# Gorilla-Lab-SCUT/DCL-Net

Hardware: AMD Instinct MI355X
Metric: frames/sec DCL_Net.forward @ YCB-V bs32 (higher is better)
Workload: dtype f32 (exact 3xbf16-split products on the bf16 MFMA, f32 accumulate)

## Files before the change

dcl-net_amd/csrc/linear_split.hip:

```cpp
#include <hip/hip_runtime.h>
#include "common.h"

namespace {

typedef float sp_f32x16 __attribute__((ext_vector_type(16)));
typedef float sp_f32x2 __attribute__((ext_vector_type(2)));
typedef __bf16 sp_bf16x2 __attribute__((ext_vector_type(2)));
typedef __bf16 sp_bf16x8 __attribute__((ext_vector_type(8)));
typedef unsigned sp_u32x4 __attribute__((ext_vector_type(4)));
typedef __attribute__((address_space(3))) void sp_lds_void_t;

constexpr int kSpKC = 16;
constexpr int kSpBM = 256, kSpBN = 128;
constexpr int kSpA = kSpBM * kSpKC * 4;
constexpr int kSpP = kSpBN * kSpKC * 2;
constexpr int kSpB = 3 * kSpP;
constexpr int kSpST = kSpA + kSpB;

__device__ __forceinline__ unsigned sp_lds_addr(const void *p) {
  return __builtin_amdgcn_readfirstlane((unsigned)(size_t)(sp_lds_void_t *)p);
}
__device__ __forceinline__ void sp_glds16(unsigned voff, const void *sbase, unsigned lds_byte_addr) {
  unsigned keep;
  asm volatile("s_mov_b32 %0, m0\n\ts_mov_b32 m0, %3\n\ts_nop 0\n\tglobal_load_lds_dwordx4 %1, %2\n\ts_mov_b32 m0, %0"
               : "=&s"(keep) : "v"(voff), "s"(sbase), "s"(lds_byte_addr) : "memory");
}
__device__ __forceinline__ unsigned sp_cvt2(float a, float b) {
  const sp_f32x2 v = {a, b};
  return __builtin_bit_cast(unsigned, __builtin_convertvector(v, sp_bf16x2));
}
__device__ __forceinline__ void sp_split2(float x0, float x1, unsigned &h, unsigned &m, unsigned &l) {
  h = sp_cvt2(x0, x1);
  float r0 = x0 - __uint_as_float(h << 16);
  asm volatile("" : "+v"(r0));
  float r1 = x1 - __uint_as_float(h & 0xffff0000u);
  asm volatile("" : "+v"(r1));
  m = sp_cvt2(r0, r1);
  float s0 = r0 - __uint_as_float(m << 16);
  asm volatile("" : "+v"(s0));
  float s1 = r1 - __uint_as_float(m & 0xffff0000u);
  asm volatile("" : "+v"(s1));
  l = sp_cvt2(s0, s1);
}
__device__ __forceinline__ sp_bf16x8 sp_bf(sp_u32x4 v) { return __builtin_bit_cast(sp_bf16x8, v); }

struct LinSplitArgs {
  const float *x;
  const unsigned char *planes;
  const float *bias;
  float *y;
  long long ldx, ldy;
  int M, N, K, relu;
  const float *roww;
  int rows_per_crop;
  long long w_stride;
  float *part;
  const float *b3;
  long long ldp;
  int xcd_remap;
};

__device__ __forceinline__ int sp_rowmap(int e, int h) { return (e & 3) + 8 * (e >> 2) + 4 * h; }

__global__ __launch_bounds__(256) void k_split_weight(const float *__restrict__ Wt, long long ldw, int K, int N, unsigned *__restrict__ planes) {
  const int ntn = (N + kSpBN - 1) / kSpBN;
  const long long pieces = (long long)(K / kSpKC) * ntn * kSpBN * 2;
  for (long long i = blockIdx.x * 256ll + threadIdx.x; i < pieces; i += (long long)gridDim.x * 256) {
    const int hs = (int)(i & 1), c = (int)((i >> 1) & (kSpBN - 1));
    const long long ct = i >> 8;
    const int kc = (int)(ct / ntn), tn = (int)(ct - (long long)kc * ntn);
    const int hh = hs ^ ((c >> 3) & 1), col = tn * kSpBN + c, k0 = kc * kSpKC + 8 * hh;
    unsigned h[4], m[4], l[4];
#pragma unroll
    for (int e = 0; e < 4; ++e) {
      const float w0 = col < N ? Wt[(size_t)(k0 + 2 * e) * ldw + col] : 0.0f, w1 = col < N ? Wt[(size_t)(k0 + 2 * e + 1) * ldw + col] : 0.0f;
      sp_split2(w0, w1, h[e], m[e], l[e]);
    }
    unsigned *dst = planes + (size_t)ct * (kSpB / 4) + (size_t)(c * 2 + hs) * 4;
#pragma unroll
    for (int e = 0; e < 4; ++e) { dst[e] = h[e]; dst[kSpP / 4 + e] = m[e]; dst[2 * (kSpP / 4) + e] = l[e]; }
  }
}

template <int EPI>
__global__ __launch_bounds__(256, 2) void k_linear_split(const LinSplitArgs a) {
  extern __shared__ __attribute__((aligned(16))) unsigned char sp_lds[];
  const int ntn = (a.N + kSpBN - 1) / kSpBN, ntm = (a.M + kSpBM - 1) / kSpBM, tiles = ntm * ntn;
  int t_lo, t_hi, t_stride;
  {
    const int id = blockIdx.x, nwg = gridDim.x;
    if ((a.xcd_remap & 1) && (nwg & 7) == 0) {
      const int xq = tiles >> 3, xr = tiles & 7, xcd = id & 7;
      const int x_lo = xcd < xr ? xcd * (xq + 1) : xr * (xq + 1) + (xcd - xr) * xq;
      t_lo = x_lo + (id >> 3);
      t_hi = x_lo + xq + (xcd < xr ? 1 : 0);
      t_stride = nwg >> 3;
    } else {
      t_lo = id; t_hi = tiles; t_stride = nwg;
    }
  }
  const int tid = threadIdx.x, lane = tid & 63, wave = __builtin_amdgcn_readfirstlane(tid >> 6);
  const int r = lane & 31, h = lane >> 5;
  const int nchunks = a.K / kSpKC;
  const int whatif = a.xcd_remap >> 1;
  const unsigned lds0 = sp_lds_addr(sp_lds);
  const size_t bstep = (size_t)ntn * kSpB;

  const int asw = (r >> 2) & 3;
  const unsigned char *afrag = sp_lds + (wave * 64 + r) * 64;
  const unsigned char *bfrag = sp_lds + kSpA + r * 32 + ((h ^ ((r >> 3) & 1)) << 4);

  for (int tile = t_lo; tile < t_hi; tile += t_stride) {
    const int tm = tile / ntn, tn = tile - tm * ntn;
    const int row0 = tm * kSpBM, col0 = tn * kSpBN;
    unsigned aoff[4];
#pragma unroll
    for (int i = 0; i < 4; ++i) {
      const int row = wave * 64 + i * 16 + (lane >> 2);
      const int p = (lane & 3) ^ ((row >> 2) & 3);
      const int srow = min(row0 + row, a.M - 1) - row0;
      aoff[i] = (unsigned)(((long long)srow * a.ldx + 4 * p) * 4);
    }
    const unsigned boff = (unsigned)tid * 16u;
    const float *abase = a.x + (size_t)row0 * a.ldx;
    const unsigned char *bbase = a.planes + (size_t)tn * kSpB;
    auto issue_piece = [&](int k, int stage) {
      const unsigned s0 = lds0 + (unsigned)(stage * kSpST);
      if (k < 3) sp_glds16(boff + (unsigned)(k * 4096), bbase, s0 + (unsigned)(kSpA + k * 4096 + wave * 1024));
      else sp_glds16(aoff[k - 3], abase, s0 + (unsigned)((wave * 64 + (k - 3) * 16) * 64));
      if (k == 6) { abase += kSpKC; bbase += bstep; }
    };
    auto issue = [&](int stage) {
#pragma unroll
      for (int k = 0; k < 7; ++k) issue_piece(k, stage);
    };
    sp_f32x16 acc[2][4];
#pragma unroll
    for (int i = 0; i < 2; ++i)
#pragma unroll
      for (int j = 0; j < 4; ++j)
#pragma unroll
        for (int e = 0; e < 16; ++e) acc[i][j][e] = 0.0f;

    dcl_lds_barrier();
    if constexpr (EPI == 1) {
      float *wl = reinterpret_cast<float *>(sp_lds + 2 * kSpST);
      const int row = row0 + tid, crop = row / a.rows_per_crop;
      wl[tid] = row < a.M ? a.roww[(size_t)crop * a.w_stride + (row - crop * a.rows_per_crop)] : 0.0f;
    }
    issue(0);
    asm volatile("s_waitcnt vmcnt(0)" ::: "memory");
    for (int c = 0; c < nchunks; ++c) {
      const int st = c & 1;
      asm volatile("s_waitcnt lgkmcnt(0)" ::: "memory");
      __builtin_amdgcn_s_barrier();
      const bool more = c + 1 < nchunks;
      const unsigned char *sa = afrag + st * kSpST, *sb = bfrag + st * kSpST;
      float4 av[2][2];
      sp_u32x4 ap[2][3], bp[4][3];
      auto read_a = [&](int i) {
#pragma unroll
        for (int q = 0; q < 2; ++q) av[i][q] = *reinterpret_cast<const float4 *>(sa + i * 32 * 64 + (((2 * h + q) ^ asw) << 4));
      };
      auto read_b = [&](int j) {
#pragma unroll
        for (int p = 0; p < 3; ++p) bp[j][p] = *reinterpret_cast<const sp_u32x4 *>(sb + p * kSpP + j * 32 * 32);
      };
      auto split_a = [&](int i, int part) {
        unsigned ph, pm, pl;
        const float4 v = av[i][part >> 1];
        if (part & 1) sp_split2(v.z, v.w, ph, pm, pl); else sp_split2(v.x, v.y, ph, pm, pl);
        ap[i][0][part] = ph; ap[i][1][part] = pm; ap[i][2][part] = pl;
      };
      read_a(0);
      read_b(0);
      read_a(1);
      if (more && !(whatif & 1)) issue(st ^ 1);
      __builtin_amdgcn_sched_barrier(0);
      if (!(whatif & 2)) {
#pragma unroll
        for (int part = 0; part < 4; ++part) split_a(0, part);
      } else {
#pragma unroll
        for (int p = 0; p < 3; ++p) ap[0][p] = sp_u32x4{__float_as_uint(av[0][0].x), __float_as_uint(av[0][0].y), __float_as_uint(av[0][1].x), __float_as_uint(av[0][1].y)};
      }
      read_b(1);
      __builtin_amdgcn_sched_barrier(0);
#pragma unroll
      for (int blk = 0; blk < 8; ++blk) {
        const int i = blk >> 2, j = blk & 3;
        acc[i][j] = __builtin_amdgcn_mfma_f32_32x32x16_bf16(sp_bf(ap[i][2]), sp_bf(bp[j][0]), acc[i][j], 0, 0, 0);
        acc[i][j] = __builtin_amdgcn_mfma_f32_32x32x16_bf16(sp_bf(ap[i][0]), sp_bf(bp[j][2]), acc[i][j], 0, 0, 0);
        acc[i][j] = __builtin_amdgcn_mfma_f32_32x32x16_bf16(sp_bf(ap[i][1]), sp_bf(bp[j][1]), acc[i][j], 0, 0, 0);
        acc[i][j] = __builtin_amdgcn_mfma_f32_32x32x16_bf16(sp_bf(ap[i][1]), sp_bf(bp[j][0]), acc[i][j], 0, 0, 0);
        acc[i][j] = __builtin_amdgcn_mfma_f32_32x32x16_bf16(sp_bf(ap[i][0]), sp_bf(bp[j][1]), acc[i][j], 0, 0, 0);
        acc[i][j] = __builtin_amdgcn_mfma_f32_32x32x16_bf16(sp_bf(ap[i][0]), sp_bf(bp[j][0]), acc[i][j], 0, 0, 0);
        if (blk < 4) {
          if (!(whatif & 2)) split_a(1, blk);
          else { ap[1][0][blk] = __float_as_uint(av[1][blk >> 1].x); ap[1][1][blk] = __float_as_uint(av[1][blk >> 1].y); ap[1][2][blk] = __float_as_uint(av[1][blk >> 1].z); }
        }
        if (blk < 2) read_b(blk + 2);
        __builtin_amdgcn_sched_barrier(0);
      }
      asm volatile("s_waitcnt vmcnt(0)" ::: "memory");
    }
    asm volatile("s_nop 15\n\ts_nop 7" ::: "memory");

    if constexpr (EPI == 0) {
      if (whatif & 4) continue;
      float *__restrict__ y = a.y;
      const bool whole = row0 + kSpBM <= a.M && col0 + kSpBN <= a.N;
      float bias[4];
#pragma unroll
      for (int j = 0; j < 4; ++j) {
        const int co = col0 + j * 32 + r;
        bias[j] = (a.bias && co < a.N) ? a.bias[co] : 0.0f;
      }
      if (whole) {
#pragma unroll
        for (int i = 0; i < 2; ++i)
#pragma unroll
          for (int j = 0; j < 4; ++j) {
            float *yp = y + (size_t)(row0 + wave * 64 + i * 32 + 4 * h) * a.ldy + (col0 + j * 32 + r);
#pragma unroll
            for (int e = 0; e < 16; ++e) {
              float v = acc[i][j][e] + bias[j];
              if (a.relu) v = fmaxf(v, 0.0f);
              __builtin_nontemporal_store(v, yp + (size_t)((e & 3) + 8 * (e >> 2)) * a.ldy);
            }
          }
      } else {
#pragma unroll
        for (int i = 0; i < 2; ++i)
#pragma unroll
          for (int j = 0; j < 4; ++j) {
            const int co = col0 + j * 32 + r;
#pragma unroll
            for (int e = 0; e < 16; ++e) {
              const int orow = row0 + wave * 64 + i * 32 + sp_rowmap(e, h);
              float v = acc[i][j][e] + bias[j];
              if (a.relu) v = fmaxf(v, 0.0f);
              if (orow < a.M && co < a.N) y[(size_t)orow * a.ldy + co] = v;
            }
          }
      }
    } else if constexpr (EPI == 3) {
      unsigned char *vp = reinterpret_cast<unsigned char *>(a.part);
      const int crop = row0 / a.rows_per_crop, key0 = row0 - crop * a.rows_per_crop;
#pragma unroll
      for (int j = 0; j < 4; ++j) {
        const int c = col0 + j * 32 + r;
        const float bias = (a.bias && c < a.N) ? a.bias[c] : 0.0f;
        const int hs = h ^ ((c >> 3) & 1);
#pragma unroll
        for (int i = 0; i < 2; ++i)
#pragma unroll
          for (int hf = 0; hf < 2; ++hf) {
            const long long ht = (long long)crop * a.ldp + ((key0 + wave * 64 + i * 32) >> 4) + hf;
// ... 51 lines not shown
            const float wv[4] = {w4.x, w4.y, w4.z, w4.w};
#pragma unroll
            for (int q = 0; q < 4; ++q) {
              float v = acc[i][j][4 * g4 + q] + bias;
              if (a.relu) v = fmaxf(v, 0.0f);
              s = __fmaf_rn(v, wv[q], s);
            }
          }
        s += __shfl_xor(s, 32, 64);
        if (h == 0) red[wave * kSpBN + cl] = s;
      }
      dcl_lds_barrier();
      {
        const int pt = tid >> 7, cl = tid & 127;
        if (col0 + cl < a.N && row0 + pt * 128 < a.M)
          a.part[(size_t)(2 * tm + pt) * a.ldp + col0 + cl] = red[(2 * pt) * kSpBN + cl] + red[(2 * pt + 1) * kSpBN + cl];
      }
    }
  }
}

DCL_HOOK_INT(g_sp_xcd, 1);

template <int EPI>
int launch_linear_split(const LinSplitArgs &a, hipStream_t stream) {
  const long long tiles = (long long)((a.M + kSpBM - 1) / kSpBM) * ((a.N + kSpBN - 1) / kSpBN);
  if (tiles > 0x7fffffffll) {
    dcl_set_error("dcl_linear_split_fwd: too many tiles");
    return DCL_EINVAL;
  }
  constexpr size_t lds = (size_t)2 * kSpST + (EPI == 1 ? (kSpBM + 4 * kSpBN) * sizeof(float) : 0);
  static bool attr_set = false;
  if (!attr_set) {
    (void)hipFuncSetAttribute((const void *)k_linear_split<EPI>, hipFuncAttributeMaxDynamicSharedMemorySize, (int)lds);
    attr_set = true;
  }
  hipLaunchKernelGGL((k_linear_split<EPI>), dim3((unsigned)tiles), dim3(256), lds, stream, a);
  return 0;
}

bool lin_split_ok(const float *x, int64_t ldx, const void *planes, int K) {
  return K >= kSpKC && K % kSpKC == 0 && ldx % 4 == 0 && ((size_t)x & 15) == 0 && ((size_t)planes & 15) == 0;
}

}

#ifdef DCL_DIAG
DCL_API void dcl_debug_linear_split_xcd_remap(int on) { g_sp_xcd = ((int)g_sp_xcd & ~1) | (on & 1); }
DCL_API void dcl_debug_linear_split_whatif(int bits) { g_sp_xcd = ((int)g_sp_xcd & 1) | (bits << 1); }
#endif

DCL_API int64_t dcl_linear_split_weight_bytes(int K, int N) {
  if (K <= 0 || N <= 0 || K % kSpKC) return 0;
  return (int64_t)(K / kSpKC) * ((N + kSpBN - 1) / kSpBN) * kSpB;
}

DCL_API int dcl_linear_split_weight(const float *Wt, int64_t ldw, int K, int N, void *planes, dclStream_t stream) {
  DCL_CHECK_ARG(Wt && planes && K > 0 && N > 0 && K % kSpKC == 0 && ldw >= N && ((size_t)planes & 15) == 0);
  const long long pieces = (long long)(K / kSpKC) * ((N + kSpBN - 1) / kSpBN) * kSpBN * 2;
  const unsigned grid = (unsigned)((pieces + 255) / 256 > 4096 ? 4096 : (pieces + 255) / 256);
  hipLaunchKernelGGL(k_split_weight, dim3(grid), dim3(256), 0, (hipStream_t)stream, Wt, (long long)ldw, K, N, (unsigned *)planes);
  DCL_LAUNCH_CHECK();
  return 0;
}

DCL_API int dcl_linear_split_fwd(const float *x, int64_t ldx, const void *planes, const float *bias, float *y, int64_t ldy, int M, int N,
                                 int K, int relu, dclStream_t stream) {
  DCL_CHECK_ARG(M >= 0 && N > 0 && K > 0 && x && planes && y && ldx >= K && ldy >= N);
  DCL_CHECK_ARG(lin_split_ok(x, ldx, planes, K));
  if (M == 0) return 0;
  LinSplitArgs a{x, (const unsigned char *)planes, bias, y, ldx, ldy, M, N, K, relu, nullptr, 1, 0, nullptr, nullptr, 0, (int)g_sp_xcd};
  int rc = launch_linear_split<0>(a, (hipStream_t)stream);
  if (rc) return rc;
  DCL_LAUNCH_CHECK();
  return 0;
}

DCL_API int dcl_linear_split_pool_fwd(const float *x, int64_t ldx, const void *planes, const float *bias, const float *roww,
                                      int rows_per_crop, int64_t w_stride, float *part, int64_t ldp, int M, int N, int K, int relu,
                                      dclStream_t stream) {
  DCL_CHECK_ARG(M > 0 && N > 0 && K > 0 && x && planes && roww && part && ldx >= K && ldp >= N && rows_per_crop >= 1 && w_stride >= 0);
  DCL_CHECK_ARG(lin_split_ok(x, ldx, planes, K));
  LinSplitArgs a{x, (const unsigned char *)planes, bias, nullptr, ldx, 0, M, N, K, relu, roww, rows_per_crop, w_stride, part, nullptr, ldp,
                 (int)g_sp_xcd};
  int rc = launch_linear_split<1>(a, (hipStream_t)stream);
  if (rc) return rc;
  DCL_LAUNCH_CHECK();
  return 0;
}

DCL_API int dcl_linear_split_vpieces_fwd(const float *x, int64_t ldx, const void *planes, const float *bias, void *vplanes,
                                         int rows_per_crop, int M, int N, int K, int relu, dclStream_t stream) {
  DCL_CHECK_ARG(M > 0 && N > 0 && N <= 320 && N % 32 == 0 && K > 0 && x && planes && vplanes && ldx >= K && rows_per_crop > 0);
  DCL_CHECK_ARG(rows_per_crop % kSpBM == 0 && M % rows_per_crop == 0 && (((size_t)vplanes) & 15) == 0);
  DCL_CHECK_ARG(lin_split_ok(x, ldx, planes, K));
  LinSplitArgs a{x, (const unsigned char *)planes, bias, nullptr, ldx, 0, M, N, K, relu, nullptr, rows_per_crop, 0, (float *)vplanes, nullptr,
                 (long long)(rows_per_crop / 16), (int)g_sp_xcd};
  int rc = launch_linear_split<3>(a, (hipStream_t)stream);
  if (rc) return rc;
  DCL_LAUNCH_CHECK();
  return 0;
}

DCL_API int dcl_linear_split_rowdot_fwd(const float *x, int64_t ldx, const void *planes, const float *bias, const float *w3, int64_t ldw3,
                                        const float *b3, float *out, int M, int N, int K, dclStream_t stream) {
  DCL_CHECK_ARG(M >= 0 && N > 0 && N <= kSpBN && K > 0 && x && planes && w3 && b3 && out && ldx >= K && ldw3 >= 1);
  DCL_CHECK_ARG(lin_split_ok(x, ldx, planes, K));
  if (M == 0) return 0;
  LinSplitArgs a{x, (const unsigned char *)planes, bias, nullptr, ldx, 0, M, N, K, 1, w3, 1, ldw3, out, b3, 0, (int)g_sp_xcd};
  int rc = launch_linear_split<2>(a, (hipStream_t)stream);
  if (rc) return rc;
  DCL_LAUNCH_CHECK();
  return 0;
}
```

dcl-net_amd/models/DCL_Net.py:

```python
from functools import partial

import numpy as np
import torch
import torch.nn as nn

from .. import ops
from .. import spconv
from ..libs.pointgroup_ops.functions import pointgroup_ops
from .losses import losses
from .Modules import (Aligner, Backbone_SPCONV, BasicBlock_3DCONV, Head_MultiLayerPerceptron,
                      Ops_GetPointFeat_spconv)

HOST_TIMES = None
_QUEUE_SHIMS = []
SIDE_STREAM_PRIORITY = -1
_SIDE_STREAMS = {}
SCALE_LISTS = [2, 4, 6, 8]
VOXEL_NUM_LIMIT = [64, 64, 64]


def normalize_vector(v):
    return v / (torch.sqrt(v.pow(2).sum(1, keepdim=True)) + 1e-8)


def ortho9d2matrix(x_raw, y_raw, z_raw):
    if not (torch.is_grad_enabled() and (x_raw.requires_grad or y_raw.requires_grad or z_raw.requires_grad)):
        return ops.ortho9d_to_matrix(torch.cat([x_raw, y_raw, z_raw], dim=1))
    dev = x_raw.device
    m = torch.stack([normalize_vector(x_raw), normalize_vector(y_raw), normalize_vector(z_raw)], dim=2).cpu()
    U, _, Vh = torch.linalg.svd(m)
    ones = torch.ones(m.shape[0], dtype=m.dtype)
    sigma = torch.diag_embed(torch.stack([ones, ones, torch.det(U @ Vh)], dim=1))
    return (U @ sigma @ Vh).to(dev)


def _mlp3(dims):
    return Head_MultiLayerPerceptron(dims, ["relu", "relu", "none"], [False] * 3, [0.0] * 3)


def _fuser():
    return Head_MultiLayerPerceptron([512, 512, 512, 1024], ["relu"] * 3, [True] * 3, [0.0] * 3)


class Network(nn.Module):
    def __init__(self, cfg, mode="train", fused=True, graph_max_batch=8, async_inputs=False, graph_max_points=98304,
                 single_stream=False, pipeline_chunks=1, capture_graph=True, pair_features=None):
        super().__init__()
        self.single_stream = bool(single_stream)
        self._pair_features = pair_features
        self.pipeline_chunks = int(pipeline_chunks)
        self.capture_graph = bool(capture_graph)
        self.graph_max_batch = int(graph_max_batch)
        self.graph_max_points = int(graph_max_points)
        self.async_inputs = bool(async_inputs)
        self.voxelization_mode = cfg.voxelization_mode
        self.unit_voxel_extent = np.array(cfg.unit_voxel_extent)
        self.mode = mode
        self.fused = fused
        self.n_inp = cfg.n_inp
        self.n_tmp = cfg.n_tmp
        self.backbone_dims = [7, 16, 32, 32, 64, 64, 128, 128, 256]
        self.backbone_stride_layers = [1, 3, 5]
        self.backbone_inp = Backbone_SPCONV(self.backbone_dims, self.backbone_stride_layers, cfg.backbone)
        self.backbone_tmp = Backbone_SPCONV(self.backbone_dims, self.backbone_stride_layers, cfg.backbone)
        self.stage1_get_point_feats = Ops_GetPointFeat_spconv(SCALE_LISTS, self.unit_voxel_extent, VOXEL_NUM_LIMIT)
        block = partial(BasicBlock_3DCONV, size=1, bias=False, stride=1, padding=0, norm=True, act="relu", drop=0.0)
        for grp in ("1", "2"):
            for side in ("Xc", "Yo"):
                for kind, d_out in (("p", 256), ("m", 64)):
                    setattr(self, "disengage_%s_%s%s" % (side, kind, grp),
# ... 303 lines not shown
        fuse_buf, conf_in = new(512), new(128)
        planes, fused = None, False
        if fuse is not None and self.mode == "test":
            b, par = fuse
            nk = self.n_inp if side == "Xc" else self.n_tmp
            nq = self.n_tmp if side == "Xc" else self.n_inp
            if rows == b * nk and nk % 256 == 0:
                planes, whole = ops.attention_planes(b, nq, nk, par, dev)
                fused = planes is not None and whole
        v1 = None if fused else new(256)
        if side == "Xc":
            return {"fuse1": fuse_buf, "conf_in1": conf_in, "Xcp1": fuse_buf[:, :256], "Xcm1": conf_in[:, :64],
                    "Xcp2": v1, "Xcm2": new(64), "planes2": planes}
        return {"fuse2": fuse_buf, "conf_in2": conf_in, "Yop2": fuse_buf[:, 256:], "Yom2": conf_in[:, 64:],
                "Yop1": v1, "Yom1": new(64), "planes1": planes}

    def _disengage(self, f, side, pf_rows, act, rows=slice(None)):
        W1t, t1, second = f["dis_" + side]
        H = self._lin_relu(pf_rows, W1t, t1)
        if pf_rows.shape[0] <= self.GROUP_ROWS:
            ops.linear_group([(H[:, 256 * j:256 * (j + 1)], second[j][0], second[j][1], True, act[side + tag][rows])
                              for j, (tag, _) in enumerate(self._DIS_TAGS)])
            return
        for j, (tag, _) in enumerate(self._DIS_TAGS):
            Wt, bias = second[j]
            Hj = H[:, 256 * j:256 * (j + 1)]
            if act[side + tag] is None:
                sw = ops.prepared_linear(Wt, Hj)
                planes = act["planes2" if side == "Xc" else "planes1"]
                all_rows = act[side + ("m2" if side == "Xc" else "m1")].shape[0]
                if sw is not None and pf_rows.shape[0] == all_rows:
                    ops.linear_split_vpieces(Hj, sw, bias, planes, self.n_inp if side == "Xc" else self.n_tmp, relu=True)
                    continue
                act[side + tag] = torch.empty((all_rows, 256), dtype=torch.float32, device=H.device)
            ops.linear(Hj, Wt, bias, True, out=act[side + tag][rows])

    def _dense(self, f, pf_inp, pf_tmp, b, dev):
        act = {}
        for side, pfs in (("Xc", pf_inp), ("Yo", pf_tmp)):
            act.update(self._disengage_buffers(side, pfs.shape[0], dev, fuse=(b, 1)))
            self._disengage(f, side, pfs, act)
        return self._dense_tail(f, act, b, dev)

    def _dense_tail(self, f, act, b, dev, side=None):
        main = torch.cuda.current_stream(dev)

        class _Both(object):
            def __enter__(self_inner):
                if side is not None:
                    side.wait_stream(main)
                    self_inner.ctx = torch.cuda.stream(side)
                    self_inner.ctx.__enter__()

            def __exit__(self_inner, *a):
                if side is not None:
                    self_inner.ctx.__exit__(*a)
        second = _Both()
        par = 2 if side is not None else 1
# ... 392 lines not shown
```

dcl-net_amd/ops.py:

```python
import ctypes as C
import threading

import weakref

import torch

from . import _native as N

_c_int = C.c_int
_c_float = C.c_float

PROFILE_EVENTS = None


def _i32_ptr_or_null(t):
    return N.ptr(t) if t is not None else N.vp(0)


def voxelize_idx(coords, batch_size, mode=4):
    if coords.is_cuda:
        raise RuntimeError("voxelize_idx is a host (DataLoader-side) op: pass a CPU tensor")
    assert coords.is_contiguous() and coords.dtype == torch.int64 and coords.dim() == 2
    n, ncol = coords.shape
    input_map = torch.zeros(n, dtype=torch.int32)
# ... 758 lines not shown
            pw >= (n + 3) // 4 * 4)


def linear_dma(x, Wt, bias=None, relu=False, out=None):
    N.need_cuda(x, Wt)
    assert x.dim() == 2 and Wt.dim() == 2 and x.shape[1] == Wt.shape[0] and x.dtype == Wt.dtype == torch.float32
    M, K = x.shape
    n = Wt.shape[1]
    if out is None:
        out = torch.empty((M, n), dtype=torch.float32, device=x.device)
    assert out.shape == (M, n) and out.dtype == torch.float32 and out.is_cuda
    for t in (x, Wt, out):
        assert t.stride(1) == 1 or t.shape[1] == 1, "rows must be dense"
    if bias is not None:
        assert bias.is_cuda and bias.dtype == torch.float32 and bias.numel() == n and bias.is_contiguous()
    pitch = lambda t: int(t.stride(0)) if t.shape[0] > 1 else max(int(t.stride(0)), int(t.shape[1]))
    N.check(N.lib().dcl_linear_dma_fwd(N.ptr(x), C.c_int64(pitch(x)), N.ptr(Wt), C.c_int64(pitch(Wt)), N.ptr(bias), N.ptr(out),
                                       C.c_int64(pitch(out)), int(M), int(n), int(K), int(bool(relu)), N.stream()), "linear_dma_fwd")
    return out


GEMM_SPLIT = True
SPLIT_MIN_TILES = 192
_PREPARED = {}


def prepare_linear(Wt):
    K, n = Wt.shape
    if not Wt.is_cuda or n <= 64 or K % 16 or K < 16:
        return None
    ent = _PREPARED.get(id(Wt))
    if ent is not None and ent[0]() is Wt:
        return ent[1]
    sw = SplitWeight(Wt)
    sw.Wt = None
    key = id(Wt)
    _PREPARED[key] = (weakref.ref(Wt, lambda _r, key=key: _PREPARED.pop(key, None)), sw)
    return sw


def prepared_linear(Wt, x):
    if not GEMM_SPLIT:
        return None
    ent = _PREPARED.get(id(Wt))
    if ent is None or ent[0]() is not Wt:
        return None
    sw = ent[1]
    M = x.shape[0]
    if ((M + 255) // 256) * ((sw.n + 127) // 128) < SPLIT_MIN_TILES or not linear_split_ok(x, sw.K):
        return None
    return sw

# ... 100 lines not shown
def linear_split_vpieces(x, sw, bias, vplanes, rows_per_crop, relu=True):
    N.need_cuda(x, vplanes)
    M, K, n = x.shape[0], sw.K, sw.n
    assert x.shape[1] == K and n <= 320 and n % 32 == 0 and rows_per_crop % 256 == 0 and M % rows_per_crop == 0
    pitch = lambda t: int(t.stride(0)) if t.shape[0] > 1 else max(int(t.stride(0)), int(t.shape[1]))
    N.check(N.lib().dcl_linear_split_vpieces_fwd(N.ptr(x), C.c_int64(pitch(x)), N.ptr(sw.planes), N.ptr(bias), N.ptr(vplanes),
                                                 int(rows_per_crop), int(M), int(n), int(K), int(bool(relu)), N.stream()),
            "linear_split_vpieces_fwd")
    return vplanes


def linear_split_rowdot(x, sw, bias, w3, b3, out=None):
    N.need_cuda(x, w3, b3)
    M, K, n = x.shape[0], sw.K, sw.n
    assert x.shape[1] == K and n <= 128 and w3.shape == (n, 1) and b3.numel() == 1 and bias.numel() == n
    if out is None:
        out = torch.empty((M, 1), dtype=torch.float32, device=x.device)
    assert out.is_contiguous() and out.numel() == M
    pitch = lambda t: int(t.stride(0)) if t.shape[0] > 1 else max(int(t.stride(0)), int(t.shape[1]))
    N.check(N.lib().dcl_linear_split_rowdot_fwd(N.ptr(x), C.c_int64(pitch(x)), N.ptr(sw.planes), N.ptr(bias), N.ptr(w3),
                                                C.c_int64(int(w3.stride(0))), N.ptr(b3), N.ptr(out), int(M), int(n), int(K), N.stream()),
            "linear_split_rowdot_fwd")
    return out


def conf_softmax(b, logit1, logit2):
    N.need_cuda(logit1, logit2)
    assert logit1.is_contiguous() and logit2.is_contiguous() and logit1.numel() % b == 0 and logit2.numel() % b == 0
    n1, n2 = logit1.numel() // b, logit2.numel() // b
    dev = logit1.device
    conf = torch.empty((b, n1 + n2), dtype=torch.float32, device=dev)
    w = torch.empty((b, n1 + n2), dtype=torch.float32, device=dev)
    ws = torch.empty((b, 2), dtype=torch.float32, device=dev)
    N.check(N.lib().dcl_conf_softmax(b, n1, n2, N.ptr(logit1), N.ptr(logit2), N.ptr(conf), N.ptr(w), N.ptr(ws), N.stream()),
            "conf_softmax")
    return conf, w, ws


def pool_finish2(part1, part2, ws, affine):
    b, c = ws.shape[0], part1.shape[1]
    s1, t1, s2, t2 = affine
    assert part1.is_contiguous() and part2.is_contiguous() and part1.shape[0] % b == 0 and part2.shape[0] % b == 0
    out = torch.empty((b, c), dtype=torch.float32, device=part1.device)
    N.check(N.lib().dcl_pool_finish2(b, c, part1.shape[0] // b, part2.shape[0] // b, N.ptr(part1), N.ptr(part2), N.ptr(ws),
                                     N.ptr(s1), N.ptr(t1), N.ptr(s2), N.ptr(t2), N.ptr(out), N.stream()), "pool_finish2")
    return out
# ... 280 lines not shown
```

include/dclnet_hip.h:

```cpp
#ifndef DCLNET_HIP_H_
#define DCLNET_HIP_H_

#include <stdint.h>

#ifdef __cplusplus
extern "C" {
#endif

#define DCL_EINVAL (-1)
typedef void *dclStream_t;

const char *dcl_last_error(void);
#define DCL_ABI_VERSION 2
int dcl_abi_version(void);

int dcl_voxelize_idx_count(const int64_t *coords_host, int n, int ncol, int batch_size, int mode,
                           int32_t *input_map_host, int32_t *n_active_host, int32_t *max_active_host);
int dcl_voxelize_idx_fill(const int64_t *coords_host, int n, int ncol, const int32_t *input_map_host,
                          int n_active, int max_active, int64_t *output_coords_host,
                          int32_t *output_map_host);
int dcl_voxelize_idx_fill_mode(const int64_t *coords_host, int n, int ncol, const int32_t *input_map_host,
                               int n_active, int max_active, int mode, int64_t *output_coords_host,
                               int32_t *output_map_host);

// ... 206 lines not shown
                         float *trans, float *R, dclStream_t stream);

int dcl_linear_fwd(const float *x, int64_t ldx, const float *Wt, int64_t ldw, const float *bias, float *y, int64_t ldy,
                   int M, int N, int K, int relu, void *workspace, int64_t workspace_bytes, dclStream_t stream);

int dcl_linear_dma_fwd(const float *x, int64_t ldx, const float *Wt, int64_t ldw, const float *bias, float *y, int64_t ldy,
                       int M, int N, int K, int relu, dclStream_t stream);
int dcl_linear_pool_fwd(const float *x, int64_t ldx, const float *Wt, int64_t ldw, const float *bias, const float *roww,
                        int rows_per_crop, int64_t w_stride, float *part, int64_t ldp, int M, int N, int K, int relu,
                        dclStream_t stream);
int dcl_linear_rowdot_fwd(const float *x, int64_t ldx, const float *Wt, int64_t ldw, const float *bias, const float *w3,
                          int64_t ldw3, const float *b3, float *out, int M, int N, int K, dclStream_t stream);
int64_t dcl_linear_split_weight_bytes(int K, int N);
int dcl_linear_split_weight(const float *Wt, int64_t ldw, int K, int N, void *planes, dclStream_t stream);
int dcl_linear_split_fwd(const float *x, int64_t ldx, const void *planes, const float *bias, float *y, int64_t ldy, int M, int N,
                         int K, int relu, dclStream_t stream);
int dcl_linear_split_pool_fwd(const float *x, int64_t ldx, const void *planes, const float *bias, const float *roww,
                              int rows_per_crop, int64_t w_stride, float *part, int64_t ldp, int M, int N, int K, int relu,
                              dclStream_t stream);
int dcl_linear_split_vpieces_fwd(const float *x, int64_t ldx, const void *planes, const float *bias, void *vplanes,
                                 int rows_per_crop, int M, int N, int K, int relu, dclStream_t stream);
int dcl_linear_split_rowdot_fwd(const float *x, int64_t ldx, const void *planes, const float *bias, const float *w3, int64_t ldw3,
                                const float *b3, float *out, int M, int N, int K, dclStream_t stream);
int dcl_conf_softmax(int b, int n1, int n2, const float *logit1, const float *logit2, float *conf, float *w, float *wsum,
                     dclStream_t stream);
int dcl_pool_finish2(int b, int c, int nslices1, int nslices2, const float *part1, const float *part2, const float *wsum,
                     const float *scale1, const float *shift1, const float *scale2, const float *shift2, float *out,
                     dclStream_t stream);

#define DCL_LINEAR_MAX_JOBS 8
typedef struct DclLinearJob {
  const float *x; int64_t ldx;
  const float *Wt; int64_t ldw;
  const float *bias;
  float *y; int64_t ldy;
  int M, N, K, relu;
} DclLinearJob;
int dcl_linear_group_fwd(const DclLinearJob *jobs, int njobs, dclStream_t stream);

int dcl_ortho9d_to_matrix(int b, const float *o9, float *R, dclStream_t stream);

int dcl_rulebook_transpose(const int32_t *nbr, int cap_out, const int32_t *n_out_dev, int n_out_host, int kvol,
                           int32_t *inv, int cap_in, dclStream_t stream);
int dcl_sparse_conv_wgrad_splits(int n_out, int32_t *splits_host);
int dcl_sparse_conv_wgrad(const float *feat, const int32_t *nbr, int cap, int n_out, const float *dout, int cin, int cout,
                          int kvol, float *partial, float *dW, dclStream_t stream);
// ... 79 lines not shown
```

Before: 2091.

## Group split-bf16 linear jobs into one launch with half-width tile path

```diff
diff --git a/dcl-net_amd/csrc/linear_split.hip b/dcl-net_amd/csrc/linear_split.hip
--- a/dcl-net_amd/csrc/linear_split.hip
+++ b/dcl-net_amd/csrc/linear_split.hip
@@ -1,4 +1,6 @@
 #include <hip/hip_runtime.h>
+#include <atomic>
+#include <type_traits>
 #include "common.h"
 
 namespace {
@@ -44,19 +46,28 @@
 }
 __device__ __forceinline__ sp_bf16x8 sp_bf(sp_u32x4 v) { return __builtin_bit_cast(sp_bf16x8, v); }
 
-struct LinSplitArgs {
+struct LinSplitJob {
   const float *x;
   const unsigned char *planes;
   const float *bias;
   float *y;
   long long ldx, ldy;
   int M, N, K, relu;
+  int rich;
+  int rows_per_crop;
   const float *roww;
-  int rows_per_crop;
   long long w_stride;
   float *part;
   const float *b3;
   long long ldp;
+  int ntm, ntn;
+};
+
+constexpr int kSpMaxJobs = DCL_LINEAR_SPLIT_MAX_JOBS;
+
+struct LinSplitGroup {
+  LinSplitJob job[kSpMaxJobs];
+  int njobs, width, tiles;
   int xcd_remap;
 };
 
@@ -83,13 +94,13 @@
 }
 
 template <int EPI>
-__global__ __launch_bounds__(256, 2) void k_linear_split(const LinSplitArgs a) {
+__global__ __launch_bounds__(256, 2) void k_linear_split(const LinSplitGroup g) {
   extern __shared__ __attribute__((aligned(16))) unsigned char sp_lds[];
-  const int ntn = (a.N + kSpBN - 1) / kSpBN, ntm = (a.M + kSpBM - 1) / kSpBM, tiles = ntm * ntn;
+  const int tiles = g.tiles;
   int t_lo, t_hi, t_stride;
   {
     const int id = blockIdx.x, nwg = gridDim.x;
-    if ((a.xcd_remap & 1) && (nwg & 7) == 0) {
+    if ((g.xcd_remap & 1) && (nwg & 7) == 0) {
       const int xq = tiles >> 3, xr = tiles & 7, xcd = id & 7;
       const int x_lo = xcd < xr ? xcd * (xq + 1) : xr * (xq + 1) + (xcd - xr) * xq;
       t_lo = x_lo + (id >> 3);
@@ -101,18 +112,33 @@
   }
   const int tid = threadIdx.x, lane = tid & 63, wave = __builtin_amdgcn_readfirstlane(tid >> 6);
   const int r = lane & 31, h = lane >> 5;
-  const int nchunks = a.K / kSpKC;
-  const int whatif = a.xcd_remap >> 1;
+  const int whatif = g.xcd_remap >> 1;
   const unsigned lds0 = sp_lds_addr(sp_lds);
-  const size_t bstep = (size_t)ntn * kSpB;
 
   const int asw = (r >> 2) & 3;
   const unsigned char *afrag = sp_lds + (wave * 64 + r) * 64;
   const unsigned char *bfrag = sp_lds + kSpA + r * 32 + ((h ^ ((r >> 3) & 1)) << 4);
 
   for (int tile = t_lo; tile < t_hi; tile += t_stride) {
-    const int tm = tile / ntn, tn = tile - tm * ntn;
+    LinSplitJob a = g.job[0];
+    int tm, tn;
+    if (g.njobs == 1) {
+      tm = tile / a.ntn;
+      tn = tile - tm * a.ntn;
+    } else {
+      tm = tile / g.width;
+      tn = tile - tm * g.width;
+      int ji = 0;
+#pragma unroll
+      for (int j = 0; j + 1 < kSpMaxJobs; ++j)
+        if (ji == j && j + 1 < g.njobs && tn >= g.job[j].ntn) { tn -= g.job[j].ntn; ji = j + 1; }
+      if (ji) a = g.job[ji];
+    }
     const int row0 = tm * kSpBM, col0 = tn * kSpBN;
+    const int nchunks = a.K / kSpKC;
+    const size_t bstep = (size_t)a.ntn * kSpB;
+    const bool half = a.N - col0 <= 2 * 32;
+    const bool rich = EPI != 0 && a.rich;
     unsigned aoff[4];
 #pragma unroll
     for (int i = 0; i < 4; ++i) {
@@ -124,15 +150,18 @@
     const unsigned boff = (unsigned)tid * 16u;
     const float *abase = a.x + (size_t)row0 * a.ldx;
     const unsigned char *bbase = a.planes + (size_t)tn * kSpB;
-    auto issue_piece = [&](int k, int stage) {
+    auto issue = [&](auto nj_c, int stage) {
+      constexpr int NJ = decltype(nj_c)::value;
       const unsigned s0 = lds0 + (unsigned)(stage * kSpST);
-      if (k < 3) sp_glds16(boff + (unsigned)(k * 4096), bbase, s0 + (unsigned)(kSpA + k * 4096 + wave * 1024));
-      else sp_glds16(aoff[k - 3], abase, s0 + (unsigned)((wave * 64 + (k - 3) * 16) * 64));
-      if (k == 6) { abase += kSpKC; bbase += bstep; }
-    };
-    auto issue = [&](int stage) {
-#pragma unroll
-      for (int k = 0; k < 7; ++k) issue_piece(k, stage);
+#pragma unroll
+      for (int k = 0; k < 7; ++k) {
+        if (k < 3) {
+          if (NJ == 4 || wave < 2) sp_glds16(boff + (unsigned)(k * 4096), bbase, s0 + (unsigned)(kSpA + k * 4096 + wave * 1024));
+        } else {
+          sp_glds16(aoff[k - 3], abase, s0 + (unsigned)((wave * 64 + (k - 3) * 16) * 64));
+        }
+      }
+      abase += kSpKC; bbase += bstep;
     };
     sp_f32x16 acc[2][4];
 #pragma unroll
@@ -143,12 +172,14 @@
         for (int e = 0; e < 16; ++e) acc[i][j][e] = 0.0f;
 
     dcl_lds_barrier();
-    if constexpr (EPI == 1) {
+    if (EPI == 1 && rich) {
       float *wl = reinterpret_cast<float *>(sp_lds + 2 * kSpST);
       const int row = row0 + tid, crop = row / a.rows_per_crop;
       wl[tid] = row < a.M ? a.roww[(size_t)crop * a.w_stride + (row - crop * a.rows_per_crop)] : 0.0f;
     }
-    issue(0);
+    auto k_loop = [&](auto nj_c) {
+    constexpr int NJ = decltype(nj_c)::value;
+    issue(nj_c, 0);
     asm volatile("s_waitcnt vmcnt(0)" ::: "memory");
     for (int c = 0; c < nchunks; ++c) {
       const int st = c & 1;
@@ -175,8 +206,26 @@
       read_a(0);
       read_b(0);
       read_a(1);
-      if (more && !(whatif & 1)) issue(st ^ 1);
+      if (more && !(whatif & 1)) issue(nj_c, st ^ 1);
       __builtin_amdgcn_sched_barrier(0);
+      if constexpr (NJ == 2) {
+#pragma unroll
+        for (int part = 0; part < 4; ++part) split_a(0, part);
+        read_b(1);
+        __builtin_amdgcn_sched_barrier(0);
+#pragma unroll
+        for (int blk = 0; blk < 4; ++blk) {
+          const int i = blk >> 1, j = blk & 1;
+          acc[i][j] = __builtin_amdgcn_mfma_f32_32x32x16_bf16(sp_bf(ap[i][2]), sp_bf(bp[j][0]), acc[i][j], 0, 0, 0);
+          acc[i][j] = __builtin_amdgcn_mfma_f32_32x32x16_bf16(sp_bf(ap[i][0]), sp_bf(bp[j][2]), acc[i][j], 0, 0, 0);
+          acc[i][j] = __builtin_amdgcn_mfma_f32_32x32x16_bf16(sp_bf(ap[i][1]), sp_bf(bp[j][1]), acc[i][j], 0, 0, 0);
+          acc[i][j] = __builtin_amdgcn_mfma_f32_32x32x16_bf16(sp_bf(ap[i][1]), sp_bf(bp[j][0]), acc[i][j], 0, 0, 0);
+          acc[i][j] = __builtin_amdgcn_mfma_f32_32x32x16_bf16(sp_bf(ap[i][0]), sp_bf(bp[j][1]), acc[i][j], 0, 0, 0);
+          acc[i][j] = __builtin_amdgcn_mfma_f32_32x32x16_bf16(sp_bf(ap[i][0]), sp_bf(bp[j][0]), acc[i][j], 0, 0, 0);
+          if (blk < 2) { split_a(1, 2 * blk); split_a(1, 2 * blk + 1); }
+          __builtin_amdgcn_sched_barrier(0);
+        }
+      } else {
       if (!(whatif & 2)) {
 #pragma unroll
         for (int part = 0; part < 4; ++part) split_a(0, part);
@@ -202,25 +251,29 @@
         if (blk < 2) read_b(blk + 2);
         __builtin_amdgcn_sched_barrier(0);
       }
+      }
       asm volatile("s_waitcnt vmcnt(0)" ::: "memory");
     }
+    };
+    if (half) k_loop(std::integral_constant<int, 2>{}); else k_loop(std::integral_constant<int, 4>{});
     asm volatile("s_nop 15\n\ts_nop 7" ::: "memory");
 
-    if constexpr (EPI == 0) {
+    if (!rich) {
       if (whatif & 4) continue;
       float *__restrict__ y = a.y;
-      const bool whole = row0 + kSpBM <= a.M && col0 + kSpBN <= a.N;
+      const int nj = half ? 2 : 4;
+      const bool whole = row0 + kSpBM <= a.M && col0 + 32 * nj <= a.N;
       float bias[4];
 #pragma unroll
       for (int j = 0; j < 4; ++j) {
         const int co = col0 + j * 32 + r;
         bias[j] = (a.bias && co < a.N) ? a.bias[co] : 0.0f;
       }
-      if (whole) {
+      auto store_blocks = [&](auto nj_c) {
 #pragma unroll
         for (int i = 0; i < 2; ++i)
 #pragma unroll
-          for (int j = 0; j < 4; ++j) {
+          for (int j = 0; j < decltype(nj_c)::value; ++j) {
             float *yp = y + (size_t)(row0 + wave * 64 + i * 32 + 4 * h) * a.ldy + (col0 + j * 32 + r);
 #pragma unroll
             for (int e = 0; e < 16; ++e) {
@@ -229,11 +282,15 @@
               __builtin_nontemporal_store(v, yp + (size_t)((e & 3) + 8 * (e >> 2)) * a.ldy);
             }
           }
+      };
+      if (whole) {
+        if (half) store_blocks(std::integral_constant<int, 2>{}); else store_blocks(std::integral_constant<int, 4>{});
       } else {
 #pragma unroll
         for (int i = 0; i < 2; ++i)
 #pragma unroll
           for (int j = 0; j < 4; ++j) {
+            if (j >= nj) continue;
             const int co = col0 + j * 32 + r;
 #pragma unroll
             for (int e = 0; e < 16; ++e) {
@@ -331,20 +388,19 @@
 
 DCL_HOOK_INT(g_sp_xcd, 1);
 
+constexpr int kSpMaxDevices = 64;
+
 template <int EPI>
-int launch_linear_split(const LinSplitArgs &a, hipStream_t stream) {
-  const long long tiles = (long long)((a.M + kSpBM - 1) / kSpBM) * ((a.N + kSpBN - 1) / kSpBN);
-  if (tiles > 0x7fffffffll) {
-    dcl_set_error("dcl_linear_split_fwd: too many tiles");
-    return DCL_EINVAL;
+int launch_linear_split(const LinSplitGroup &g, hipStream_t stream) {
+  constexpr size_t lds = (size_t)2 * kSpST + (EPI == 1 ? (kSpBM + 4 * kSpBN) * sizeof(float) : 0);
+  static std::atomic<bool> attr_set[kSpMaxDevices];
+  int dev = 0;
+  const bool known = hipGetDevice(&dev) == hipSuccess && dev >= 0 && dev < kSpMaxDevices;
+  if (!known || !attr_set[dev].load(std::memory_order_acquire)) {
+    (void)hipFuncSetAttribute((const void *)k_linear_split<EPI>, hipFuncAttributeMaxDynamicSharedMemorySize, (int)lds);
+    if (known) attr_set[dev].store(true, std::memory_order_release);
   }
-  constexpr size_t lds = (size_t)2 * kSpST + (EPI == 1 ? (kSpBM + 4 * kSpBN) * sizeof(float) : 0);
-  static bool attr_set = false;
-  if (!attr_set) {
-    (void)hipFuncSetAttribute((const void *)k_linear_split<EPI>, hipFuncAttributeMaxDynamicSharedMemorySize, (int)lds);
-    attr_set = true;
-  }
-  hipLaunchKernelGGL((k_linear_split<EPI>), dim3((unsigned)tiles), dim3(256), lds, stream, a);
+  hipLaunchKernelGGL((k_linear_split<EPI>), dim3((unsigned)g.tiles), dim3(256), lds, stream, g);
   return 0;
 }
 
@@ -373,52 +429,97 @@
   return 0;
 }
 
-DCL_API int dcl_linear_split_fwd(const float *x, int64_t ldx, const void *planes, const float *bias, float *y, int64_t ldy, int M, int N,
-                                 int K, int relu, dclStream_t stream) {
-  DCL_CHECK_ARG(M >= 0 && N > 0 && K > 0 && x && planes && y && ldx >= K && ldy >= N);
-  DCL_CHECK_ARG(lin_split_ok(x, ldx, planes, K));
-  if (M == 0) return 0;
-  LinSplitArgs a{x, (const unsigned char *)planes, bias, y, ldx, ldy, M, N, K, relu, nullptr, 1, 0, nullptr, nullptr, 0, (int)g_sp_xcd};
-  int rc = launch_linear_split<0>(a, (hipStream_t)stream);
+static int lin_split_group(const DclLinearSplitJob *jobs, int njobs, dclStream_t stream, const char *who) {
+  LinSplitGroup g{};
+  int n = 0, epi = 0;
+  for (int q = 0; q < njobs; ++q) {
+    const DclLinearSplitJob &j = jobs[q];
+    DCL_CHECK_ARG(j.M >= 0 && j.N > 0 && j.K > 0 && j.x && j.planes && j.ldx >= j.K && lin_split_ok(j.x, j.ldx, j.planes, j.K));
+    DCL_CHECK_ARG(j.epi >= DCL_SPLIT_EPI_STORE && j.epi <= DCL_SPLIT_EPI_VPIECES);
+    LinSplitJob d{};
+    d.x = j.x; d.planes = (const unsigned char *)j.planes; d.bias = j.bias; d.ldx = j.ldx;
+    d.M = j.M; d.N = j.N; d.K = j.K; d.relu = j.relu; d.rich = j.epi != DCL_SPLIT_EPI_STORE; d.rows_per_crop = 1;
+    switch (j.epi) {
+      case DCL_SPLIT_EPI_STORE:
+        DCL_CHECK_ARG(j.y && j.ldy >= j.N);
+        d.y = j.y; d.ldy = j.ldy;
+        break;
+      case DCL_SPLIT_EPI_POOL:
+        DCL_CHECK_ARG(j.M > 0 && j.roww && j.out && j.ldp >= j.N && j.rows_per_crop >= 1 && j.w_stride >= 0);
+        d.roww = j.roww; d.rows_per_crop = j.rows_per_crop; d.w_stride = j.w_stride; d.part = (float *)j.out; d.ldp = j.ldp;
+        break;
+      case DCL_SPLIT_EPI_ROWDOT:
+        DCL_CHECK_ARG(j.N <= kSpBN && j.roww && j.b3 && j.out && j.w_stride >= 1);
+        d.relu = 1; d.roww = j.roww; d.w_stride = j.w_stride; d.part = (float *)j.out; d.b3 = j.b3;
+        break;
+      default:
+        DCL_CHECK_ARG(j.M > 0 && j.N <= 320 && j.N % 32 == 0 && j.out && j.rows_per_crop > 0);
+        DCL_CHECK_ARG(j.rows_per_crop % kSpBM == 0 && j.M % j.rows_per_crop == 0 && (((size_t)j.out) & 15) == 0);
+        d.rows_per_crop = j.rows_per_crop; d.part = (float *)j.out; d.ldp = j.rows_per_crop / 16;
+        break;
+    }
+    if (j.epi != DCL_SPLIT_EPI_STORE) {
+      DCL_CHECK_ARG(epi == 0 || epi == j.epi);
+      epi = j.epi;
+    }
+    DCL_CHECK_ARG(j.M == jobs[0].M);
+    d.ntm = (j.M + kSpBM - 1) / kSpBM; d.ntn = (j.N + kSpBN - 1) / kSpBN;
+    g.width += d.ntn;
+    g.job[n++] = d;
+  }
+  if (jobs[0].M == 0) return 0;
+  const long long tiles = (long long)g.job[0].ntm * g.width;
+  if (tiles > 0x7fffffffll) {
+    dcl_set_error("%s: too many tiles", who);
+    return DCL_EINVAL;
+  }
+  g.njobs = n; g.tiles = (int)tiles;
+  g.xcd_remap = (int)g_sp_xcd;
+  const hipStream_t st = (hipStream_t)stream;
+  int rc = epi == DCL_SPLIT_EPI_POOL     ? launch_linear_split<1>(g, st)
+           : epi == DCL_SPLIT_EPI_ROWDOT ? launch_linear_split<2>(g, st)
+           : epi == DCL_SPLIT_EPI_VPIECES ? launch_linear_split<3>(g, st)
+                                           : launch_linear_split<0>(g, st);
   if (rc) return rc;
   DCL_LAUNCH_CHECK();
   return 0;
 }
 
+DCL_API int dcl_linear_split_group_fwd(const DclLinearSplitJob *jobs, int njobs, dclStream_t stream) {
+  DCL_CHECK_ARG(jobs && njobs >= 1 && njobs <= kSpMaxJobs);
+  return lin_split_group(jobs, njobs, stream, __func__);
+}
+
+DCL_API int dcl_linear_split_fwd(const float *x, int64_t ldx, const void *planes, const float *bias, float *y, int64_t ldy, int M, int N,
+                                 int K, int relu, dclStream_t stream) {
+  DCL_CHECK_ARG(M >= 0 && y);
+  DclLinearSplitJob j{};
+  j.x = x; j.ldx = ldx; j.planes = planes; j.bias = bias; j.M = M; j.N = N; j.K = K; j.relu = relu; j.epi = DCL_SPLIT_EPI_STORE;
+  j.y = y; j.ldy = ldy;
+  return lin_split_group(&j, 1, stream, __func__);
+}
+
 DCL_API int dcl_linear_split_pool_fwd(const float *x, int64_t ldx, const void *planes, const float *bias, const float *roww,
                                       int rows_per_crop, int64_t w_stride, float *part, int64_t ldp, int M, int N, int K, int relu,
                                       dclStream_t stream) {
-  DCL_CHECK_ARG(M > 0 && N > 0 && K > 0 && x && planes && roww && part && ldx >= K && ldp >= N && rows_per_crop >= 1 && w_stride >= 0);
-  DCL_CHECK_ARG(lin_split_ok(x, ldx, planes, K));
-  LinSplitArgs a{x, (const unsigned char *)planes, bias, nullptr, ldx, 0, M, N, K, relu, roww, rows_per_crop, w_stride, part, nullptr, ldp,
-                 (int)g_sp_xcd};
-  int rc = launch_linear_split<1>(a, (hipStream_t)stream);
-  if (rc) return rc;
-  DCL_LAUNCH_CHECK();
-  return 0;
+  DclLinearSplitJob j{};
+  j.x = x; j.ldx = ldx; j.planes = planes; j.bias = bias; j.M = M; j.N = N; j.K = K; j.relu = relu; j.epi = DCL_SPLIT_EPI_POOL;
+  j.roww = roww; j.rows_per_crop = rows_per_crop; j.w_stride = w_stride; j.out = part; j.ldp = ldp;
+  return lin_split_group(&j, 1, stream, __func__);
 }
 
 DCL_API int dcl_linear_split_vpieces_fwd(const float *x, int64_t ldx, const void *planes, const float *bias, void *vplanes,
                                          int rows_per_crop, int M, int N, int K, int relu, dclStream_t stream) {
-  DCL_CHECK_ARG(M > 0 && N > 0 && N <= 320 && N % 32 == 0 && K > 0 && x && planes && vplanes && ldx >= K && rows_per_crop > 0);
-  DCL_CHECK_ARG(rows_per_crop % kSpBM == 0 && M % rows_per_crop == 0 && (((size_t)vplanes) & 15) == 0);
-  DCL_CHECK_ARG(lin_split_ok(x, ldx, planes, K));
-  LinSplitArgs a{x, (const unsigned char *)planes, bias, nullptr, ldx, 0, M, N, K, relu, nullptr, rows_per_crop, 0, (float *)vplanes, nullptr,
-                 (long long)(rows_per_crop / 16), (int)g_sp_xcd};
-  int rc = launch_linear_split<3>(a, (hipStream_t)stream);
-  if (rc) return rc;
-  DCL_LAUNCH_CHECK();
-  return 0;
+  DclLinearSplitJob j{};
+  j.x = x; j.ldx = ldx; j.planes = planes; j.bias = bias; j.M = M; j.N = N; j.K = K; j.relu = relu; j.epi = DCL_SPLIT_EPI_VPIECES;
+  j.rows_per_crop = rows_per_crop; j.out = vplanes;
+  return lin_split_group(&j, 1, stream, __func__);
 }
 
 DCL_API int dcl_linear_split_rowdot_fwd(const float *x, int64_t ldx, const void *planes, const float *bias, const float *w3, int64_t ldw3,
                                         const float *b3, float *out, int M, int N, int K, dclStream_t stream) {
-  DCL_CHECK_ARG(M >= 0 && N > 0 && N <= kSpBN && K > 0 && x && planes && w3 && b3 && out && ldx >= K && ldw3 >= 1);
-  DCL_CHECK_ARG(lin_split_ok(x, ldx, planes, K));
-  if (M == 0) return 0;
-  LinSplitArgs a{x, (const unsigned char *)planes, bias, nullptr, ldx, 0, M, N, K, 1, w3, 1, ldw3, out, b3, 0, (int)g_sp_xcd};
-  int rc = launch_linear_split<2>(a, (hipStream_t)stream);
-  if (rc) return rc;
-  DCL_LAUNCH_CHECK();
-  return 0;
-}
+  DclLinearSplitJob j{};
+  j.x = x; j.ldx = ldx; j.planes = planes; j.bias = bias; j.M = M; j.N = N; j.K = K; j.relu = 1; j.epi = DCL_SPLIT_EPI_ROWDOT;
+  j.roww = w3; j.w_stride = ldw3; j.b3 = b3; j.out = out;
+  return lin_split_group(&j, 1, stream, __func__);
+}
diff --git a/dcl-net_amd/models/DCL_Net.py b/dcl-net_amd/models/DCL_Net.py
--- a/dcl-net_amd/models/DCL_Net.py
+++ b/dcl-net_amd/models/DCL_Net.py
@@ -44,8 +44,9 @@
 
 class Network(nn.Module):
     def __init__(self, cfg, mode="train", fused=True, graph_max_batch=8, async_inputs=False, graph_max_points=98304,
-                 single_stream=False, pipeline_chunks=1, capture_graph=True, pair_features=None):
+                 single_stream=False, pipeline_chunks=1, capture_graph=True, pair_features=None, group_split=True):
         super().__init__()
+        self.group_split = bool(group_split)
         self.single_stream = bool(single_stream)
         self._pair_features = pair_features
         self.pipeline_chunks = int(pipeline_chunks)
@@ -395,18 +396,30 @@
             ops.linear_group([(H[:, 256 * j:256 * (j + 1)], second[j][0], second[j][1], True, act[side + tag][rows])
                               for j, (tag, _) in enumerate(self._DIS_TAGS)])
             return
+        jobs = []
         for j, (tag, _) in enumerate(self._DIS_TAGS):
             Wt, bias = second[j]
             Hj = H[:, 256 * j:256 * (j + 1)]
+            sw = ops.prepared_linear(Wt, Hj)
             if act[side + tag] is None:
-                sw = ops.prepared_linear(Wt, Hj)
                 planes = act["planes2" if side == "Xc" else "planes1"]
                 all_rows = act[side + ("m2" if side == "Xc" else "m1")].shape[0]
                 if sw is not None and pf_rows.shape[0] == all_rows:
-                    ops.linear_split_vpieces(Hj, sw, bias, planes, self.n_inp if side == "Xc" else self.n_tmp, relu=True)
+                    jobs.append(("vpieces", Hj, sw, bias, True, planes, self.n_inp if side == "Xc" else self.n_tmp))
                     continue
                 act[side + tag] = torch.empty((all_rows, 256), dtype=torch.float32, device=H.device)
-            ops.linear(Hj, Wt, bias, True, out=act[side + tag][rows])
+            if sw is not None and not ops.VENDOR_GEMM:
+                jobs.append(("store", Hj, sw, bias, True, act[side + tag][rows]))
+            else:
+                jobs.append((Hj, Wt, bias, act[side + tag][rows]))
+        if self.group_split and all(isinstance(job[0], str) for job in jobs):
+            ops.linear_split_group(jobs)
+            return
+        for job in jobs:
+            if isinstance(job[0], str):
+                ops.linear_split_group([job])
+            else:
+                ops.linear(job[0], job[1], job[2], True, out=job[3])
 
     def _dense(self, f, pf_inp, pf_tmp, b, dev):
         act = {}
diff --git a/dcl-net_amd/ops.py b/dcl-net_amd/ops.py
--- a/dcl-net_amd/ops.py
+++ b/dcl-net_amd/ops.py
@@ -804,12 +804,13 @@
 
 GEMM_SPLIT = True
 SPLIT_MIN_TILES = 192
+SPLIT_MIN_COLS = 64
 _PREPARED = {}
 
 
 def prepare_linear(Wt):
     K, n = Wt.shape
-    if not Wt.is_cuda or n <= 64 or K % 16 or K < 16:
+    if not Wt.is_cuda or n < SPLIT_MIN_COLS or K % 16 or K < 16:
         return None
     ent = _PREPARED.get(id(Wt))
     if ent is not None and ent[0]() is Wt:
@@ -956,6 +957,71 @@
                                                 C.c_int64(int(w3.stride(0))), N.ptr(b3), N.ptr(out), int(M), int(n), int(K), N.stream()),
             "linear_split_rowdot_fwd")
     return out
+
+
+class _SplitJob(C.Structure):
+    _fields_ = [("x", C.c_void_p), ("ldx", C.c_int64), ("planes", C.c_void_p), ("bias", C.c_void_p),
+                ("M", C.c_int32), ("N", C.c_int32), ("K", C.c_int32), ("relu", C.c_int32), ("epi", C.c_int32),
+                ("rows_per_crop", C.c_int32), ("y", C.c_void_p), ("ldy", C.c_int64), ("roww", C.c_void_p), ("w_stride", C.c_int64),
+                ("out", C.c_void_p), ("ldp", C.c_int64), ("b3", C.c_void_p)]
+
+
+LINEAR_SPLIT_GROUP_MAX = 4
+
+
+def linear_split_group(jobs):
+    assert 1 <= len(jobs) <= LINEAR_SPLIT_GROUP_MAX and len({int(job[1].shape[0]) for job in jobs}) == 1, "one row count per launch"
+    arr = (_SplitJob * len(jobs))()
+    outs, keep = [], []
+    pitch = lambda t: int(t.stride(0)) if t.shape[0] > 1 else max(int(t.stride(0)), int(t.shape[1]))
+    for q, job in zip(arr, jobs):
+        kind, x, sw, bias = job[:4]
+        N.need_cuda(x)
+        assert x.dim() == 2 and x.shape[1] == sw.K and x.dtype == torch.float32 and (x.stride(1) == 1 or x.shape[1] == 1)
+        M, K, n = x.shape[0], sw.K, sw.n
+        if bias is not None:
+            assert bias.is_cuda and bias.dtype == torch.float32 and bias.numel() == n and bias.is_contiguous()
+        q.x, q.ldx, q.planes, q.bias = x.data_ptr(), pitch(x), sw.planes.data_ptr(), (None if bias is None else bias.data_ptr())
+        q.M, q.N, q.K, q.relu, q.rows_per_crop = int(M), int(n), int(K), 1, 1
+        if kind == "store":
+            relu, out = job[4:]
+            if out is None:
+                out = torch.empty((M, n), dtype=torch.float32, device=x.device)
+            assert out.shape == (M, n) and out.dtype == torch.float32 and out.is_cuda and (out.stride(1) == 1 or n == 1)
+            q.epi, q.relu, q.y, q.ldy = 0, int(bool(relu)), out.data_ptr(), pitch(out)
+        elif kind == "vpieces":
+            relu, out, rows_per_crop = job[4:]
+            N.need_cuda(out)
+            assert n <= 320 and n % 32 == 0 and rows_per_crop % 256 == 0 and M % rows_per_crop == 0
+            q.epi, q.relu, q.out, q.rows_per_crop = 3, int(bool(relu)), out.data_ptr(), int(rows_per_crop)
+        elif kind == "rowdot":
+            w3, b3, out = job[4:]
+            N.need_cuda(w3, b3)
+            assert n <= 128 and w3.shape == (n, 1) and b3.numel() == 1 and bias is not None
+            if out is None:
+                out = torch.empty((M, 1), dtype=torch.float32, device=x.device)
+            assert out.is_contiguous() and out.numel() == M
+            q.epi, q.roww, q.w_stride, q.b3, q.out = 2, w3.data_ptr(), int(w3.stride(0)), b3.data_ptr(), out.data_ptr()
+            keep.append((w3, b3))
+        else:
+            assert kind == "pool", kind
+            relu, roww, out, rows_per_crop, w_stride = job[4:]
+            N.need_cuda(roww)
+            if rows_per_crop is None:
+                rows_per_crop, w_stride = M, 0
+                assert roww.is_contiguous() and roww.numel() == M
+            assert roww.dtype == torch.float32 and M % rows_per_crop == 0
+            tiles = (M + LINEAR_POOL_TILE - 1) // LINEAR_POOL_TILE
+            if out is None:
+                out = torch.empty((tiles, n), dtype=torch.float32, device=x.device)
+            assert out.shape == (tiles, n) and out.stride(1) == 1
+            q.epi, q.relu, q.roww, q.rows_per_crop, q.w_stride = 1, int(bool(relu)), roww.data_ptr(), int(rows_per_crop), int(w_stride)
+            q.out, q.ldp = out.data_ptr(), pitch(out)
+            keep.append(roww)
+        outs.append(out)
+        keep.append((x, sw, bias))
+    N.check(N.lib().dcl_linear_split_group_fwd(arr, len(jobs), N.stream()), "linear_split_group_fwd")
+    return outs
 
 
 def conf_softmax(b, logit1, logit2):
diff --git a/include/dclnet_hip.h b/include/dclnet_hip.h
--- a/include/dclnet_hip.h
+++ b/include/dclnet_hip.h
@@ -252,6 +252,23 @@
                                  int rows_per_crop, int M, int N, int K, int relu, dclStream_t stream);
 int dcl_linear_split_rowdot_fwd(const float *x, int64_t ldx, const void *planes, const float *bias, const float *w3, int64_t ldw3,
                                 const float *b3, float *out, int M, int N, int K, dclStream_t stream);
+#define DCL_LINEAR_SPLIT_MAX_JOBS 4
+#define DCL_SPLIT_EPI_STORE 0
+#define DCL_SPLIT_EPI_POOL 1
+#define DCL_SPLIT_EPI_ROWDOT 2
+#define DCL_SPLIT_EPI_VPIECES 3
+typedef struct DclLinearSplitJob {
+  const float *x; int64_t ldx;
+  const void *planes;
+  const float *bias;
+  int M, N, K, relu;
+  int epi, rows_per_crop;
+  float *y; int64_t ldy;
+  const float *roww; int64_t w_stride;
+  void *out; int64_t ldp;
+  const float *b3;
+} DclLinearSplitJob;
+int dcl_linear_split_group_fwd(const DclLinearSplitJob *jobs, int njobs, dclStream_t stream);
 int dcl_conf_softmax(int b, int n1, int n2, const float *logit1, const float *logit2, float *conf, float *w, float *wsum,
                      dclStream_t stream);
 int dcl_pool_finish2(int b, int c, int nslices1, int nslices2, const float *part1, const float *part2, const float *wsum,
```

New measurement: 2099 (median of 6 runs). No clear change (+0.4%).
